# ergodicio/tsadar

Hardware: AMD Instinct MI355X
Metric: spectra/sec (fwd+grad), 1024-lambda EPW+IAW form factor, batch 4096 (higher is better)
Workload: dtype f64

## Files before the change

tsadar_amd/csrc/k_spectrum_fused.inc:

```

template <int NI, int GM, bool ZH, bool FAR = false>
__device__ __forceinline__ double point_fused(const Base& b, const Base& bn, bool has_next, const LineS<NI>& L, const Tables& T,
                                              double PQ, double cw, BaseAdj& ba, double& xen, double& Fn, LineS<NI>& J) {
  PointF<NI> pf;
  point_core<NI, ZH, FAR>(b, bn, has_next, L, T, pf);
  const double ik2 = pf.ik2, ike2 = pf.ike2, vph = pf.vph, gsum = pf.gsum, Wl = pf.Wl, dW = pf.dW, idx = pf.idx, D = pf.D;
  const double cer = pf.cer, cei = pf.cei, opc = pf.opc, cim = pf.cim, er = pf.er, ei = pf.ei, ieps2 = pf.ieps2, ce2 = pf.ce2, ci2 = pf.ci2;
  const double N = pf.N, t1 = pf.t1, S = pf.S, dop = pf.dop;
  const double* xi = pf.xi; const double* zr = pf.zr; const double* zi = pf.zi; const double* dzr = pf.dzr; const double* dzi = pf.dzi;
  const double* hk = pf.hk; const double* gs = pf.gs;
  const double Sb = PQ * dop;
  const double PSQ = PQ * S;
  const double fwd = S * dop;
  J.wL = __builtin_fma(PSQ * b.wd, cw, J.wL);
  const double Nb = Sb * t1;
  const double ikb0 = Sb * N * ieps2;
  const double e2 = -2.0 * (ikb0 * t1);
  const double NbI = Nb * L.ivTe;
  const double ci2b2 = 2.0 * (NbI * b.F);
  ba.F = NbI * ci2;
  J.ivTe += (Nb * ci2) * b.F;
  const double erb = e2 * er, eib = e2 * ei;
  double cerb = erb, ceib = eib, cimb = eib;
  if (!FAR) {
    const double ce2b2 = 2.0 * (Nb * gsum);
    cerb = erb + ce2b2 * cer; ceib = eib + ce2b2 * cei;
    cimb = eib + ci2b2 * cim;
  }
  const double creb = erb + ci2b2 * opc;
  const double cp = ceib * kPi;
  const double ike2b = cp * D - cerb * Wl;
  const double Wlb = -cerb * ike2;
  ba.xe = Wlb * dW;
  if (GM == 1) {
    double Wml, dWm;
    w_lookup(T.Wm, b.xe, Wml, dWm);
    J.m += Wlb * Wml;
  }
  Fn = (cp * ike2) * idx;
  ba.F -= Fn;
  xen = -Fn * D;
  ba.xe -= xen;
  double k2acc = 0.0, vphb = 0.0;
  const double u = FAR ? 0.0 : Nb * ce2;
#pragma unroll
  for (int s = 0; s < NI; ++s) {
    double w, xib;
    if (FAR) {
      w = creb * zr[s];
      xib = hk[s] * (creb * dzr[s]);
    } else {
      const double v = u * gs[s];
      J.cs[s] += v;
      w = creb * zr[s] + cimb * zi[s];
      xib = -2.0 * (v * xi[s] * L.cs[s]) + hk[s] * (creb * dzr[s] + cimb * dzi[s]);
    }
    const double wk = w * ik2;
    J.a_i[s] += wk;
    k2acc += wk * hk[s];
    vphb += xib * L.ixi[s];
    J.ixi[s] += xib * vph;
  }
  const double we = ike2b * ik2;
  J.a_e += we;
  ba.k2 = -k2acc - we * ike2;
  ba.wd = PSQ * L.i2wL + vphb * b.ik;
  ba.ik = ikb0 + vphb * b.wd;
  return fwd;
}

struct KsAcc { double p1a, p2a, p1b, p2b; };

template <int NI, int GM>
__device__ __forceinline__ double base_reverse_fused(const Base& b, const LineS<NI>& L, const Tables& T, const BaseAdj& ba,
                                                     LineS<NI>& LB) {
  const double Hb = ba.F * b.F;
  if (GM == 1) {
    Tables Tm = T;
    Tm.hc = T.hcm;
    double Hm, dHm;
    hermite_lookup_c(Tm, b.xe, Hm, dHm);
    LB.m += (b.xe < T.vx0 || b.xe > T.vxlast) ? 0.0 : Hb * Hm;
  }
  const double xeb = ba.xe + Hb * b.dH;
  const double vph = b.wd * b.ik, k = b.k2 * b.ik;
  const double vphb = xeb * L.ivTe;
  LB.Ud -= vphb;
  LB.ivTe += xeb * (vph - L.Ud);
  const double wdb = ba.wd + vphb * b.ik;
  const double ikb = ba.ik + vphb * b.wd;
  LB.wL -= wdb;
  LB.Vd -= wdb * k;
  const double kb = wdb * L.Vd + ikb * (b.ik * b.ik);
  return 2.0 * ba.k2 - kb * b.ik;
}

template <int NI, int GM>
__device__ __forceinline__ double base_reverse_xf(const Base& b, const LineS<NI>& L, const Tables& T, double xeb_in, double Fb,
                                                  LineS<NI>& LB) {
  const double Hb = Fb * b.F;
  if (GM == 1) {
    Tables Tm = T;
    Tm.hc = T.hcm;
    double Hm, dHm;
    hermite_lookup_c(Tm, b.xe, Hm, dHm);
    LB.m += (b.xe < T.vx0 || b.xe > T.vxlast) ? 0.0 : Hb * Hm;
  }
  const double xeb = xeb_in + Hb * b.dH;
  const double vph = b.wd * b.ik, k = b.k2 * b.ik;
  const double vphb = xeb * L.ivTe;
  LB.Ud -= vphb;
  LB.ivTe += xeb * (vph - L.Ud);
  const double wdb = vphb * b.ik;
  const double ikb = vphb * b.wd;
  LB.wL -= wdb;
  LB.Vd -= wdb * k;
  const double kb = wdb * L.Vd + ikb * (b.ik * b.ik);
  return -kb * b.ik;
}

#ifdef TSFF_TRACE
__device__ unsigned long long* g_trace_buf = nullptr;
#define TSFF_STAMP(k) do { if (tid == 0 && g_trace_buf) g_trace_buf[(size_t)item * 16 + (k)] = wall_clock64(); } while (0)
#define TSFF_STAMP_WAVE(k) do { if (lane == 0 && g_trace_buf) g_trace_buf[(size_t)item * 16 + (k) + hw] = wall_clock64(); } while (0)
#define TSFF_STAMP_HW() do { if (tid == 0 && g_trace_buf) g_trace_buf[(size_t)item * 16] = ((unsigned long long)__builtin_amdgcn_s_getreg(20 | (31 << 11)) << 32) | (unsigned)__builtin_amdgcn_s_getreg(4 | (31 << 11)); } while (0)
#else
#define TSFF_STAMP(k) do {} while (0)
#define TSFF_STAMP_WAVE(k) do {} while (0)
#define TSFF_STAMP_HW() do {} while (0)
#endif
typedef const double __attribute__((address_space(4))) cdouble_t;
template <int DIR>
__device__ __forceinline__ void conv4_phase(const double* __restrict__ xs, int Ls, int sl, cdouble_t* pt, int na, double (&acc)[4]) {
  const double* __restrict__ X0 = xs + sl, * __restrict__ X1 = X0 + Ls, * __restrict__ X2 = X1 + Ls, * __restrict__ X3 = X2 + Ls;
  double V0 = X0[0], V1 = X1[0], V2 = X2[0];
#pragma unroll 2
  for (int a = 0; a < na; ++a) {
    const double V3 = X3[a], V4 = X0[a + 1], V5 = X1[a + 1], V6 = X2[a + 1];
    const double g0 = pt[4 * DIR * a], g1 = pt[4 * DIR * a + DIR], g2 = pt[4 * DIR * a + 2 * DIR], g3 = pt[4 * DIR * a + 3 * DIR];
    acc[0] = __builtin_fma(g3, V3, __builtin_fma(g2, V2, __builtin_fma(g1, V1, __builtin_fma(g0, V0, acc[0]))));
    acc[1] = __builtin_fma(g3, V4, __builtin_fma(g2, V3, __builtin_fma(g1, V2, __builtin_fma(g0, V1, acc[1]))));
    acc[2] = __builtin_fma(g3, V5, __builtin_fma(g2, V4, __builtin_fma(g1, V3, __builtin_fma(g0, V2, acc[2]))));
    acc[3] = __builtin_fma(g3, V6, __builtin_fma(g2, V5, __builtin_fma(g1, V4, __builtin_fma(g0, V3, acc[3]))));
    V0 = V4; V1 = V5; V2 = V6;
  }
}

constexpr int kRedSums = 32;
#ifndef TSFF_FUSED_FAR
#define TSFF_FUSED_FAR 1
#endif
template <int NI, int GM, bool ZH, bool EX = false>
__global__ __launch_bounds__(kHalf, 2) void k_spectrum_fused(KStatic S, KCall K, int f0, int flags,
                                                             const double* __restrict__ lrec) {
  const bool use_ks = flags & 2, interleaved = flags & 4;
  const int item = blockIdx.x;
  const int f_il = interleaved ? (int)(item >= K.B) : 0;
  const int b = K.b0 + item - f_il * K.B, tid = threadIdx.x;
  const size_t gitem = (size_t)f_il * K.Btot + b;
  constexpr int TPF = kHalf, NW = TPF / 64;
  const int ht = tid, lane = tid & 63, hw = tid >> 6;
  const int f = __builtin_amdgcn_readfirstlane(interleaved ? f_il : f0);
  extern __shared__ __align__(16) unsigned char smem[];
  TSFF_STAMP_HW();
  TSFF_STAMP(1);
  const Smem m = carve(smem, S, 1, GM, use_ks, true, ZH, EX);
  constexpr int NPk = TSFF_NP(NI);
  const double* __restrict__ xpar = K.params + (size_t)b * S.NP;
  const int npts = S.npts, NA = S.n_angles;
  const int hs = S.hs, Ls = npts / 4 + 2 * hs;
  double* xs = m.x;
  auto XA = [&](int j) { return (j & 3) * Ls + (j >> 2) + hs; };
  Tables T;
  const double lam_shift = S.lam_shift[f];
  const double* __restrict__ omgs = S.omgs[f];
  constexpr int kPair = 2;
  const int jp[2] = {kPair * ht, npts / 2 + kPair * ht};
  double ws[2][kPair + 1];
  LineS<NI> L;
  double* __restrict__ ksc = use_ks ? m.ksc : nullptr;
  {
    TSFF_STAGE_LOCALS;
    stage_issue(TSFF_STAGE_ARGS, m, S, K, S.shared_fe ? 0 : b, ZH, f);
    stage_commit(TSFF_STAGE_ARGS, m, S, K, S.shared_fe ? 0 : b, T, ZH, f);
#pragma unroll
    for (int p = 0; p < 2; ++p)
#pragma unroll
      for (int q = 0; q <= kPair; ++q) ws[p][q] = omgs[min(jp[p] + q, npts - 1)];
    {
      lines_load<NI>(lrec + gitem * kLineRec, 1, [](double v) { return uni(v); }, L);
    }
    if (use_ks) {
#pragma unroll
      for (int p = 0; p < 2; ++p)
#pragma unroll
        for (int q = 0; q <= kPair; ++q) ksc[min(jp[p] + q, npts - 1)] = ks_eval(ws[p][q], L.wpe2);
    }
    for (int i = ht; i < 8 * hs; i += TPF) { const int ph_ = i / (2 * hs), o = i - ph_ * 2 * hs; xs[ph_ * Ls + (o < hs ? o : Ls - 2 * hs + o)] = 0.0; }
    if (ht < 2) xs[4 * Ls + ht] = 0.0;
  }
  double w_lo[2], w_hi[2];
#pragma unroll
  for (int p = 0; p < 2; ++p) {
    w_lo[p] = __hiloint2double(__builtin_amdgcn_readlane(__double2hiint(ws[p][0]), 0), __builtin_amdgcn_readlane(__double2loint(ws[p][0]), 0));
    w_hi[p] = __hiloint2double(__builtin_amdgcn_readlane(__double2hiint(ws[p][kPair]), 63), __builtin_amdgcn_readlane(__double2loint(ws[p][kPair]), 63));
  }
  const bool far0 = TSFF_FUSED_FAR && far_range_w<NI>(w_lo[0], w_hi[0], L), far1 = TSFF_FUSED_FAR && far_range_w<NI>(w_lo[1], w_hi[1], L);
  const double ex_wse = ((lane >> 4) & 1) ? w_hi[1] : w_hi[0];
  __syncthreads();
  TSFF_STAMP(2);
  auto JQ = [&](int q) { return jp[q >> 1] + (q & 1); };
  LineS<NI> J[kStrip];
  KsAcc KA[kStrip];
  double xa[kStrip];
#pragma unroll
  for (int q = 0; q < kStrip; ++q) { zero_lines<NI>(J[q]); xa[q] = 0.0; KA[q].p1a = KA[q].p2a = KA[q].p1b = KA[q].p2b = 0.0; }
  const double cw = -0.5 * L.i2wL * L.i2wL;
  double* exl = m.ex;
  double* exb = EX ? m.ex + kExComp * kHalf : nullptr;
  if (EX) {
    const int Pb = (lane >> 4) & 1, ab = lane & 15;
    if (lane < 32 && ab < NA) {
      const double wse = ex_wse;
      Base be;
      base_eval<NI>(wse, ks_eval(wse, L.wpe2), m.cosa[ab], L, T, be);
      double* o = exb + 16 * (2 * hw + Pb) + ab;
      o[0] = be.wd; o[kExBound] = be.ik; o[2 * kExBound] = be.xe; o[3 * kExBound] = be.F; o[4 * kExBound] = be.dH;
    }
    __builtin_amdgcn_fence(__ATOMIC_RELEASE, "wavefront");
    __builtin_amdgcn_wave_barrier();
  }
  auto sweep = [&](auto pair_tag, auto far_tag) {
    constexpr int P = decltype(pair_tag)::value;
    constexpr bool FAR = decltype(far_tag)::value;
    const int jb = jp[P];
    const int j2 = min(jb + kPair, npts - 1);
    const double ks2 = EX ? (use_ks ? ksc[j2] : ks_eval(ws[P][kPair], L.wpe2)) : 0.0;
    double ct_n = m.cosa[0], wa_n = m.wsa[0];
    for (int a = 0; a < NA; ++a) {
      const double ct = uni(ct_n), wa = uni(wa_n * L.pref);
      { const int an = min(a + 1, NA - 1); ct_n = m.cosa[an]; wa_n = m.wsa[an]; }
      Base b0;
      base_eval<NI>(ws[P][0], use_ks ? ksc[jb] : ks_eval(ws[P][0], L.wpe2), ct, L, T, b0);
      if (EX) {
        exl[ht] = b0.wd; exl[kHalf + ht] = b0.ik; exl[2 * kHalf + ht] = b0.xe; exl[3 * kHalf + ht] = b0.F; exl[4 * kHalf + ht] = b0.dH;
        __builtin_amdgcn_fence(__ATOMIC_RELEASE, "wavefront");
        __builtin_amdgcn_wave_barrier();
      }
#pragma unroll
      for (int i = 0; i < kPair; ++i) {
        constexpr int q0 = kPair * P;
        const int q = q0 + i, j = jb + i;
        const bool has_next = (j + 1) < npts;
        Base b1;
        if (EX && i == kPair - 1) {
          __builtin_amdgcn_wave_barrier();
          __builtin_amdgcn_fence(__ATOMIC_ACQUIRE, "wavefront");
          const double* src = lane == 63 ? exb + 16 * (2 * hw + P) + a : exl + ht + 1;
          const int cs = lane == 63 ? kExBound : kHalf;
          b1.wd = src[0]; b1.ik = src[cs]; b1.xe = src[2 * cs]; b1.F = src[3 * cs]; b1.dH = src[4 * cs];
          b1.ks = ks2;
          b1.k2 = base_k2<NI>(ks2, ct, L);
          __builtin_amdgcn_wave_barrier();
        } else {
          base_eval<NI>(ws[P][i + 1], use_ks ? ksc[min(j + 1, npts - 1)] : ks_eval(ws[P][i + 1], L.wpe2), ct, L, T, b1);
        }
        BaseAdj ba;
        double xen, Fn;
        xa[q] = __builtin_fma(wa, point_fused<NI, GM, ZH, FAR>(b0, b1, has_next, L, T, wa, cw, ba, xen, Fn, J[q]), xa[q]);
        const double k22a = base_reverse_fused<NI, GM>(b0, L, T, ba, J[q]);
        const double k22b = base_reverse_xf<NI, GM>(b1, L, T, xen, Fn, J[q]);
        KA[q].p1a += k22a; KA[q].p2a = __builtin_fma(k22a, ct, KA[q].p2a);
        KA[q].p1b += k22b; KA[q].p2b = __builtin_fma(k22b, ct, KA[q].p2b);
        b0 = b1;
      }
    }
  };
  if (far0) sweep(std::integral_constant<int, 0>{}, std::true_type{}); else sweep(std::integral_constant<int, 0>{}, std::false_type{});
  if (far1) sweep(std::integral_constant<int, 1>{}, std::true_type{}); else sweep(std::integral_constant<int, 1>{}, std::false_type{});
  TSFF_STAMP_WAVE(9);
#ifdef TSFF_SWEEP_ONLY
  {
    double acc = 0.0;
#pragma unroll
    for (int q = 0; q < kStrip; ++q) acc += xa[q] + J[q].wL + J[q].ivTe + J[q].a_e + J[q].Ud + J[q].Vd + J[q].ixi[0] + J[q].a_i[0] + J[q].cs[0] + KA[q].p1a + KA[q].p2a + KA[q].p1b + KA[q].p2b;
    __syncthreads();
    TSFF_STAMP(3);
    if (acc == 1.2345e300) K.gpart[0] = acc;
    TSFF_STAMP(8);
    return;
  }
#endif
#pragma unroll
  for (int q = 0; q < kStrip; ++q) {
    const int j = JQ(q);
    const double ksa = use_ks ? ksc[j] : ks_eval(ws[q >> 1][q & 1], L.wpe2);
    const double ksb = use_ks ? ksc[min(j + 1, npts - 1)] : ks_eval(ws[q >> 1][(q & 1) + 1], L.wpe2);
    const double p1 = KA[q].p1a + KA[q].p1b;
    J[q].kL = L.kL * p1 - (ksa * KA[q].p2a + ksb * KA[q].p2b);
    J[q].wpe2 = -(0.5 / (kC * kC)) * (p1 - L.kL * (KA[q].p2a / ksa + KA[q].p2b / ksb));
  }
  {
    const bool filt = f == TSFF_FEATURE_ELE && S.filt;
#pragma unroll
    for (int q = 0; q < kStrip; ++q) {
      const double w = ws[q >> 1][q & 1];
      xs[XA(JQ(q))] = xa[q] * (filt ? w * w * S.filt[JQ(q)] : w * w);
    }
  }
  __syncthreads();
  TSFF_STAMP(3);

  constexpr int BPT = 4;
  typedef const double __attribute__((address_space(4))) cdouble;
  const bool raw = S.raw[f];
  const size_t row4 = (size_t)b * TSFF_NBINS + 4 * ht;
  double dpre[BPT], npre[BPT], lpre[BPT];
  uint8_t mpre[BPT];
#pragma unroll
  for (int r = 0; r < BPT; ++r) {
    dpre[r] = K.data[f][row4 + r];
    npre[r] = K.noise[f] ? K.noise[f][row4 + r] : 0.0;
    lpre[r] = f == TSFF_FEATURE_ELE ? S.lam_bin[f][4 * ht + r] : 0.0;
    mpre[r] = S.mask[f][4 * ht + r];
  }
  const double amps = raw ? 1.0 : K.amps[f][b];
  const double* __restrict__ lrp = lrec + gitem * kLineRec + 9 + 4 * NI;
  const double p_lam_v = lrp[0], p_amp1_v = lrp[1], p_amp2_v = lrp[2], p_amp3_v = lrp[3];
  double wpre[BPT];
  {
    const bool filt = f == TSFF_FEATURE_ELE && S.filt;
#pragma unroll
    for (int r = 0; r < BPT; ++r) {
      const double w = omgs[4 * ht + r];
      wpre[r] = filt ? w * w * S.filt[4 * ht + r] : w * w;
    }
  }
  double ybin[BPT] = {0.0, 0.0, 0.0, 0.0};
  conv4_phase<1>(xs, Ls, ht + S.cf_a0[f] + hs, (cdouble_t*)(S.ptaps[f] + S.cf_i0[f]), S.cf_na[f], ybin);
  double M = ybin[0];
  int pstar = 4 * ht;
#pragma unroll
  for (int r = 1; r < BPT; ++r)
    if (ybin[r] > M) { M = ybin[r]; pstar = 4 * ht + r; }
  half_argmax<NW>(M, pstar, m.red, 0, hw, lane);
  TSFF_STAMP(4);
  const double invM = raw ? 1.0 : 1.0 / M;
  const double p_lam = uni(p_lam_v), p_amp1 = uni(p_amp1_v), p_amp2 = uni(p_amp2_v), p_amp3 = uni(p_amp3_v);
  double Tb[BPT], Ap[BPT];
  double s0 = 0.0, s1 = 0.0;
#pragma unroll
  for (int r = 0; r < BPT; ++r) {
    const int pb = 4 * ht + r;
    const double A = bin_amplitude(f, raw, amps, lpre[r], p_lam, p_amp1, p_amp2, p_amp3);
    Ap[r] = A;
    const double t = thry_value(A, ybin[r], invM, K.noise[f] != nullptr, npre[r]);
    if (K.thry[f]) K.thry[f][(size_t)b * TSFF_NBINS + pb] = t;
    Tb[r] = bin_loss(S, K, f, dpre[r], t, mpre[r], s0, s1);
  }

  double sn = 0.0, a1b = 0.0, a2b = 0.0;
#pragma unroll
  for (int r = 0; r < BPT; ++r) norm_adjoint_bin(f, Tb[r], ybin[r], invM, Ap[r], amps, lpre[r], p_lam, sn, a1b, a2b);
  {
    double v5[5] = {s0, s1, sn, a1b, a2b};
#pragma unroll
    for (int k = 0; k < 5; ++k) v5[k] = wave_sum(v5[k]);
    if (lane == 0) {
#pragma unroll
      for (int k = 0; k < 5; ++k) m.red[kRedSums + k * NW + hw] = v5[k];
    }
  }
#pragma unroll
  for (int r = 0; r < BPT; ++r) xs[XA(4 * ht + r)] = Tb[r] * Ap[r] * invM;
  __syncthreads();
  TSFF_STAMP(5);
  double sx[4] = {0.0, 0.0, 0.0, 0.0};
  conv4_phase<-1>(xs, Ls, ht + S.ca_a0[f] + hs, (cdouble_t*)(S.ptaps[f] + S.ca_i0[f]), S.ca_na[f], sx);

  __syncthreads();
  TSFF_STAMP(6);
  {
    const double* r = m.red + kRedSums;
    s0 = (r[0] + r[1]) + (r[2] + r[3]);
    s1 = (r[NW] + r[NW + 1]) + (r[NW + 2] + r[NW + 3]);
    sn = (r[2 * NW] + r[2 * NW + 1]) + (r[2 * NW + 2] + r[2 * NW + 3]);
    a1b = (r[3 * NW] + r[3 * NW + 1]) + (r[3 * NW + 2] + r[3 * NW + 3]);
    a2b = (r[4 * NW] + r[4 * NW + 1]) + (r[4 * NW + 2] + r[4 * NW + 3]);
  }
  if (ht == 0) {
    if (f == TSFF_FEATURE_ELE) { K.lpart[(size_t)b * 3 + 1] = s0; K.lpart[(size_t)b * 3 + 2] = s1; }
    else K.lpart[(size_t)b * 3 + 0] = s0;
  }
  if (raw) sn = a1b = a2b = 0.0;
  {
    const bool filt = f == TSFF_FEATURE_ELE && S.filt;
    const double cn = sn * invM;
    const int s_first = 4 * ht - pstar - S.toff[f], nt = S.ntaps[f];
#pragma unroll
    for (int r = 0; r < 4; ++r) {
      const int i = 4 * ht + r, st = s_first + r;
      const double xb = (st >= 0 && st < nt) ? __builtin_fma(-cn, m.taps[3 + st], sx[r]) : sx[r];
      xs[XA(i)] = xb * wpre[r];
    }
  }
  __syncthreads();
  constexpr int NLB = 9 + 3 * NI;
  LineS<NI> LB;
  zero_lines<NI>(LB);
#pragma unroll
  for (int q = 0; q < kStrip; ++q) {
    const double xb = xs[XA(JQ(q))];
    LB.wpe2 += xb * J[q].wpe2; LB.wL += xb * J[q].wL; LB.kL += xb * J[q].kL; LB.ivTe += xb * J[q].ivTe;
    LB.a_e += xb * J[q].a_e; LB.Ud += xb * J[q].Ud; LB.Vd += xb * J[q].Vd; LB.m += xb * J[q].m;
    LB.pref += xb * xa[q];
#pragma unroll
    for (int s = 0; s < NI; ++s) { LB.ixi[s] += xb * J[q].ixi[s]; LB.a_i[s] += xb * J[q].a_i[s]; LB.cs[s] += xb * J[q].cs[s]; }
  }
  LB.pref *= 1.0 / L.pref;
#pragma unroll
  for (int s = 0; s < NI; ++s) LB.a_i[s] *= -0.5;
  {
    double lb[kLBRec];
    lines_adj_store<NI>(LB, lb);
#pragma unroll
    for (int k = 0; k < NLB; ++k) lb[k] = wave_sum(lb[k]);
    lb[NLB] = a1b; lb[NLB + 1] = a2b;
    const size_t nitems = (size_t)K.Btot * (interleaved ? 2 : 1);
    double mine = 0.0;
#pragma unroll
    for (int k = 0; k < NLB + 2; ++k) mine = lane == k ? lb[k] : mine;
    if (lane < NLB + 2) K.lbrec[((size_t)lane * NW + hw) * nitems + gitem] = mine;
  }
  TSFF_STAMP(8);
}

template <int NI>
__global__ __launch_bounds__(64) void k_fused_prep(KStatic S, const double* __restrict__ params, int B, int f0, int nload,
                                                   double* __restrict__ lrec, double* __restrict__ finrec) {
  constexpr int NPk = TSFF_NP(NI);
  const int item = blockIdx.x * 64 + threadIdx.x;
  if (item >= B * nload) return;
  const size_t nitems = (size_t)B * nload;
  const int l = item / B, b = item - l * B, f = nload == 2 ? l : f0;
  const double* __restrict__ x = params + (size_t)b * S.NP;
  double sgv[NPk];
#pragma unroll
  for (int s = 0; s < NPk; ++s) sgv[s] = S.p_sig[s] ? sigmoid(x[s]) : 0.0;
  Phys<NI> p;
  load_phys<NI>(x, S.p_scale, S.p_shift, S.p_sig, S.ti_same, true, p, sgv);
  LineS<NI> L;
  make_lines<NI>(p, S.lam_shift[f], 0, 1, L);
  {
    double ph[NPk + 1];
    phys_to_array<NI>(p, ph);
    double* __restrict__ q = finrec + item;
#pragma unroll
    for (int k = 0; k <= NPk; ++k) q[(size_t)k * nitems] = ph[k];
#pragma unroll
    for (int k = 0; k < NPk; ++k) q[(size_t)(NPk + 1 + k) * nitems] = sgv[k];
    lines_store<NI>(L, q + (size_t)(2 * NPk + 1) * nitems, nitems);
  }
  double* __restrict__ r = lrec + (size_t)item * kLineRec;
  lines_store<NI>(L, r, 1);
  r[9 + 4 * NI] = p.lam; r[10 + 4 * NI] = p.amp1; r[11 + 4 * NI] = p.amp2; r[12 + 4 * NI] = p.amp3;
}

template <int NI>
__global__ __launch_bounds__(kThreads) void k_fused_finish(KStatic S, const double* __restrict__ finrec, const double* __restrict__ lbrec,
                                                     const double* __restrict__ lpart, int B, int f0, int nload, int gm,
                                                     const uint8_t* __restrict__ gmask, double* __restrict__ grad,
                                                     double* __restrict__ loss_out, const int* __restrict__ act, int n_act,
                                                     long B_global, long b_off, double* __restrict__ packed) {
  constexpr int NPk = TSFF_NP(NI), NLB = 9 + 3 * NI, NW = kHalf / 64;
  __shared__ double red[8];
  const int lane = threadIdx.x;
  const int per_wg = kThreads / nload;
  if (blockIdx.x == gridDim.x - 1) {
    double a[3] = {0.0, 0.0, 0.0};
    constexpr int U = 8;
    for (int b0 = threadIdx.x; b0 < B; b0 += U * kThreads) {
      double v[U][3];
#pragma unroll
      for (int u = 0; u < U; ++u) {
        const int bb = b0 + u * kThreads;
#pragma unroll
        for (int k = 0; k < 3; ++k) v[u][k] = bb < B ? lpart[(size_t)bb * 3 + k] : 0.0;
      }
#pragma unroll
      for (int u = 0; u < U; ++u)
        if (b0 + u * kThreads < B) { a[0] += v[u][0]; a[1] += v[u][1]; a[2] += v[u][2]; }
    }
    double* out = packed ? packed : loss_out;
    for (int k = 0; k < 3; ++k) {
      const double v = block_sum(a[k], red);
      if (threadIdx.x == 0) out[k] = v;
    }
    return;
  }
  const int b = blockIdx.x * per_wg + lane / nload, l = nload == 2 ? (lane & 1) : 0;
  int actv[NPk];
#pragma unroll
  for (int k = 0; k < NPk; ++k) actv[k] = (packed && k < n_act) ? act[k] : -1;
  const size_t nitems = (size_t)B * nload;
  double gv[NPk];
#pragma unroll
  for (int s = 0; s < NPk; ++s) gv[s] = 0.0;
  if (b < B) {
    const int f = nload == 2 ? l : f0;
    const size_t item = (size_t)l * B + b;
    const double* __restrict__ q = finrec + item;
    double ph[NPk + 1], sgv[NPk];
#pragma unroll
    for (int k = 0; k <= NPk; ++k) ph[k] = q[(size_t)k * nitems];
#pragma unroll
    for (int k = 0; k < NPk; ++k) sgv[k] = q[(size_t)(NPk + 1 + k) * nitems];
    Phys<NI> p;
    phys_from_lds<NI>(ph, p);
    q += (size_t)(2 * NPk + 1) * nitems;
    LineS<NI> L;
    lines_load<NI>(q, nitems, [](double v) { return v; }, L);
    double lb[NLB];
#pragma unroll
    for (int k = 0; k < NLB; ++k) {
      const double* __restrict__ r = lbrec + (size_t)k * NW * nitems + item;
      lb[k] = (r[0] + r[nitems]) + (r[2 * nitems] + r[3 * nitems]);
    }
    const double a1b = lbrec[(size_t)NLB * NW * nitems + item], a2b = lbrec[(size_t)(NLB + 1) * NW * nitems + item];
    LineS<NI> LB;
    zero_lines<NI>(LB);
    lines_adj_load<NI>(lb, true, LB);
    double g[NPk];
#pragma unroll
    for (int s = 0; s < NPk; ++s) g[s] = 0.0;
    make_lines_adjoint<NI>(p, S.lam_shift[f], 0, 1, L, LB, g);
    amp_adjoint(f, a1b, a2b, g);
    tie_renorm_adjoint<NI>(S, p, gm == 1, g);
#pragma unroll
    for (int s = 0; s < NPk; ++s) gv[s] = activation_adjoint(g[s], S.p_scale[s], S.p_sig[s], [&] { return sgv[s]; }, gmask[s]);
  }
  if (nload == 2) {
#pragma unroll
    for (int s = 0; s < NPk; ++s) {
      const double o = __shfl_xor(gv[s], 1, 64);
      gv[s] = (lane & 1) ? 0.0 : gv[s] + o;
    }
  }
  if (b < B && l == 0) {
    if (packed) {
#pragma unroll
      for (int k = 0; k < NPk; ++k) {
        double v = 0.0;
#pragma unroll
        for (int s = 0; s < NPk; ++s) v = actv[k] == s ? gv[s] : v;
        if (actv[k] >= 0) packed[3 + (size_t)k * B_global + b_off + b] = v;
      }
    } else {
#pragma unroll
      for (int s = 0; s < NPk; ++s) grad[(size_t)b * NPk + s] = gv[s];
    }
  }
  if (packed) {
    const long n = (long)n_act * B_global;
    if ((long)B < B_global)
      for (long i = (long)blockIdx.x * kThreads + lane; i < n; i += (long)(gridDim.x - 1) * kThreads) {
        const long k = i / B_global, bl = i - k * B_global - b_off;
        if (bl < 0 || bl >= B) packed[3 + i] = 0.0;
      }
  }
}
```

tsadar_amd/csrc/tsff_device.h:

```cpp
#pragma once
#include <hip/hip_runtime.h>
#include <stdint.h>
#include <type_traits>

#include "../../include/tsff.h"

#ifndef TSFF_BRANCHFREE
#define TSFF_BRANCHFREE 1
#endif

namespace tsff {

constexpr int kThreads = 256;
constexpr int kStrip = 4;
constexpr int kNP_MAX = TSFF_NP(TSFF_MAX_ION);

constexpr double kC = 2.99792458e10;
constexpr double kMe = 510.9896 / (kC * kC);
constexpr double kMp = kMe * 1836.1;
constexpr double kRe = 2.8179e-13;
constexpr double kPi = 3.14159265358979323846;
constexpr double kEsq = kMe * kC * kC * kRe;
constexpr double kC0sq = 4.0 * kPi * kEsq / kMe;
constexpr double kOmgLnum = 2.0 * kPi * 1e7 * kC;
constexpr double kInvSqrt2Pi = 0.39894228040143267794;
constexpr double kSqrt2 = 1.41421356237309504880;

constexpr double kXi2_0 = -8.2;
constexpr double kXi2_h = 0.01;
constexpr double kXi2_ih = 100.0;
constexpr int kNXi2 = TSFF_NXI2;
constexpr int kNXi1 = TSFF_NXI1;

#ifndef TSFF_NEWTON
#define TSFF_NEWTON 1
#endif
__device__ __forceinline__ double frcp(double x) {
  double y = __builtin_amdgcn_rcp(x);
  double e = __builtin_fma(-x, y, 1.0);
  y = __builtin_fma(y, e, y);
#if TSFF_NEWTON > 1
  e = __builtin_fma(-x, y, 1.0);
  y = __builtin_fma(y, e, y);
#endif
  return y;
}

__device__ __forceinline__ void fsqrt2(double x, double& s, double& is) {
  const double y = __builtin_amdgcn_rsq(x);
  double g = x * y, h = 0.5 * y;
  double r = __builtin_fma(-h, g, 0.5);
  g = __builtin_fma(g, r, g);
  h = __builtin_fma(h, r, h);
#if TSFF_NEWTON > 1
  r = __builtin_fma(-h, g, 0.5);
  g = __builtin_fma(g, r, g);
  h = __builtin_fma(h, r, h);
#endif
  const double d = __builtin_fma(-g, g, x);
  s = __builtin_fma(d, h, g);
  is = h + h;
}

__device__ __forceinline__ double uni(double x) {
  const int lo = __builtin_amdgcn_readfirstlane(__double2loint(x));
  const int hi = __builtin_amdgcn_readfirstlane(__double2hiint(x));
  return __hiloint2double(hi, lo);
}

__device__ __forceinline__ double wave_sum(double v) {
#pragma unroll
  for (int o = 32; o > 0; o >>= 1) v += __shfl_xor(v, o, 64);
  return v;
}

__device__ __forceinline__ double block_sum(double v, double* scratch) {
  v = wave_sum(v);
  const int lane = threadIdx.x & 63, w = threadIdx.x >> 6;
  __syncthreads();
  if (lane == 0) scratch[w] = v;
  __syncthreads();
  return (scratch[0] + scratch[1]) + (scratch[2] + scratch[3]);
}

__device__ __forceinline__ void block_argmax(double& v, int& idx, double* scratch) {
#pragma unroll
  for (int o = 32; o > 0; o >>= 1) {
    double ov = __shfl_xor(v, o, 64);
    int oi = __shfl_xor(idx, o, 64);
    if (ov > v || (ov == v && oi < idx)) { v = ov; idx = oi; }
  }
  const int lane = threadIdx.x & 63, w = threadIdx.x >> 6;
  __syncthreads();
  if (lane == 0) { scratch[w] = v; scratch[4 + w] = (double)idx; }
  __syncthreads();
  v = scratch[0]; idx = (int)scratch[4];
#pragma unroll
  for (int k = 1; k < 4; ++k) {
    double ov = scratch[k]; int oi = (int)scratch[4 + k];
    if (ov > v || (ov == v && oi < idx)) { v = ov; idx = oi; }
  }
}

struct Tables {
  const double2* zp;
  const double* W;
  const double2* ht;
  const double2* hc;
  const double2* hcm;
  const double* Wm;
  double* Wb;
  double* Hy;
  double* Hs;
  double vx0, dv, idv, vxlast;
  double u0, utop;
  const double* etab;
  int nvx;
};
__device__ __forceinline__ void tables_set_grid(Tables& T, double vx0, double dv, int nvx) {
  T.vx0 = vx0; T.dv = dv; T.idv = 1.0 / dv; T.vxlast = vx0 + (nvx - 1) * dv; T.nvx = nvx;
  T.u0 = -vx0 * T.idv; T.utop = (double)(nvx - 1) * (1.0 - 1.1102230246251565e-16);
}

struct FeAcc {
  int iw, ih;
  double w0, w1, y0, y1, s0, s1;
};
__device__ __forceinline__ void fe_acc_init(FeAcc& a) { a.iw = a.ih = -1; a.w0 = a.w1 = a.y0 = a.y1 = a.s0 = a.s1 = 0.0; }
__device__ __forceinline__ void fe_flush_w(FeAcc& a, double* Wb) {
  if (a.iw >= 0) { atomicAdd(&Wb[a.iw], a.w0); atomicAdd(&Wb[a.iw + 1], a.w1); }
  a.w0 = a.w1 = 0.0;
}
__device__ __forceinline__ void fe_flush_h(FeAcc& a, double* Hy, double* Hs) {
  if (a.ih >= 0) {
    atomicAdd(&Hy[a.ih], a.y0); atomicAdd(&Hy[a.ih + 1], a.y1);
    atomicAdd(&Hs[a.ih], a.s0); atomicAdd(&Hs[a.ih + 1], a.s1);
  }
  a.y0 = a.y1 = a.s0 = a.s1 = 0.0;
}
__device__ __forceinline__ void fe_add_w(FeAcc& a, double* Wb, double xe, double wb) {
  const double xlast = kXi2_0 + (kNXi2 - 1) * kXi2_h;
  const double u = (xe - kXi2_0) * kXi2_ih;
  int i = (int)u;
  i = i < 0 ? 0 : (i > kNXi2 - 2 ? kNXi2 - 2 : i);
  double t = (xe - (kXi2_0 + i * kXi2_h)) * kXi2_ih;
  t = xe < kXi2_0 ? 0.0 : (xe > xlast ? 1.0 : t);
  if (i != a.iw) { fe_flush_w(a, Wb); a.iw = i; }
  a.w0 += wb * (1.0 - t);
  a.w1 += wb * t;
}
__device__ __forceinline__ void fe_add_h(FeAcc& a, const Tables& T, double x, double hb) {
  if (x < T.vx0 || x > T.vxlast) return;
  const double u = (x - T.vx0) * T.idv;
  int i = (int)u;
  i = i < 0 ? 0 : (i > T.nvx - 2 ? T.nvx - 2 : i);
  const double t = (x - (T.vx0 + i * T.dv)) * T.idv;
  if (i != a.ih) { fe_flush_h(a, T.Hy, T.Hs); a.ih = i; }
  const double t2 = t * t, t3 = t2 * t;
  a.y0 += hb * (2.0 * t3 - 3.0 * t2 + 1.0);
  a.y1 += hb * (3.0 * t2 - 2.0 * t3);
  a.s0 += hb * (t3 - 2.0 * t2 + t) * T.dv;
  a.s1 += hb * (t3 - t2) * T.dv;
}

__device__ __forceinline__ void w_lookup(const double* W, double xe, double& w, double& dw) {
#pragma clang fp contract(off)
  constexpr double kTop = (double)(kNXi2 - 1) * (1.0 - 1.1102230246251565e-16);
  const double u = __builtin_fma(xe, kXi2_ih, -kXi2_0 * kXi2_ih);
  const double uc = fmin(fmax(u, 0.0), kTop);
  const double fl = __builtin_floor(uc);
  const double t = uc - fl;
  const int i = (int)fl;
  const double a = W[i], b = W[i + 1];
  const double d = b - a;
  w = __builtin_fma(t, d, a);
  dw = (u == uc) ? d * kXi2_ih : 0.0;
}

__device__ __forceinline__ void hermite_coeffs(double2 a, double2 b, double dv, double2& c01, double2& c23) {
  const double f0 = a.x, f1 = b.x, m0 = a.y * dv, m1 = b.y * dv;
  c01 = make_double2(f0, m0);
  c23 = make_double2(-3.0 * f0 + 3.0 * f1 - 2.0 * m0 - m1, 2.0 * f0 - 2.0 * f1 + m0 + m1);
}

__device__ __forceinline__ void hermite_lookup_c(const Tables& T, double x, double& H, double& dH) {
#pragma clang fp contract(off)
  const double u = __builtin_fma(x, T.idv, T.u0);
  const double uc = fmin(fmax(u, 0.0), T.utop);
  const double fl = __builtin_floor(uc);
  const double t = uc - fl;
  const int i = (int)fl;
  const double2 c01 = T.hc[2 * i], c23 = T.hc[2 * i + 1];
  const bool out = u != uc;
  const double Hi = __builtin_fma(t, __builtin_fma(t, __builtin_fma(t, c23.y, c23.x), c01.y), c01.x);
  const double dHi = __builtin_fma(t, __builtin_fma(3.0 * t, c23.y, 2.0 * c23.x), c01.y) * T.idv;
  H = out ? -50.0 : Hi;
  dH = out ? 0.0 : dHi;
}

__device__ __forceinline__ void hermite_lookup(const Tables& T, double x, double& H, double& dH) {
  double u = (x - T.vx0) * T.idv;
  int i = (int)u;
  i = i < 0 ? 0 : (i > T.nvx - 2 ? T.nvx - 2 : i);
  const double t = (x - (T.vx0 + i * T.dv)) * T.idv;
  const double2 a = T.ht[i], b = T.ht[i + 1];
  const double f0 = a.x, f1 = b.x, m0 = a.y * T.dv, m1 = b.y * T.dv;
  const double c2 = -3.0 * f0 + 3.0 * f1 - 2.0 * m0 - m1;
  const double c3 = 2.0 * f0 - 2.0 * f1 + m0 + m1;
  if (x < T.vx0 || x > T.vxlast) { H = -50.0; dH = 0.0; }
  else {
    H = f0 + t * (m0 + t * (c2 + t * c3));
    dH = (m0 + t * (2.0 * c2 + 3.0 * t * c3)) * T.idv;
  }
}

template <int NI>
struct Phys {
  double Te, ne, m, lam, amp1, amp2, amp3, neg, teg, ud, Va;
  double Ti[NI], Z[NI], A[NI], fr[NI];
  double fsum;
};

template <int NI>
struct LineS {
  double wpe2, wL, kL, ivTe, a_e, pref, Ud, Vd;
  double i2wL;
  double m;
  double ixi[NI], a_i[NI], cs[NI];
  double hai[NI];
};

__device__ __forceinline__ double grad_coef(int g, int G) {
  return G == 1 ? -1.0 / 200.0 : -1.0 / 200.0 + (double)g / (100.0 * (double)(G - 1));
}

template <int NI>
__device__ __forceinline__ void make_lines(const Phys<NI>& p, double lam_shift, int g, int G, LineS<NI>& L) {
  const double cg = grad_coef(g, G);
  const double ne_g = 1.0e20 * p.ne * (1.0 + p.neg * cg);
  const double Te_g = p.Te * (1.0 + p.teg * cg);
  L.wL = kOmgLnum / (p.lam + lam_shift);
  L.i2wL = 2.0 / L.wL;
  L.m = 0.0;
  L.wpe2 = kC0sq * ne_g;
  L.kL = sqrt(L.wL * L.wL - L.wpe2) / kC;
  L.ivTe = 1.0 / sqrt(Te_g / kMe);
  L.a_e = L.wpe2 * L.ivTe * L.ivTe;
  L.pref = kRe * kRe * ne_g / (2.0 * kPi * kC);
  L.Ud = p.ud * 1e6;
  L.Vd = p.Va * 1e6;
  double Zbar = 0.0;
#pragma unroll
  for (int s = 0; s < NI; ++s) Zbar += p.Z[s] * p.fr[s];
#pragma unroll
  for (int s = 0; s < NI; ++s) {
    const double Ms = p.A[s] * kMp;
    const double vTi = sqrt(p.Ti[s] / Ms);
    L.ixi[s] = 1.0 / (kSqrt2 * vTi);
    L.a_i[s] = kC0sq * kMe * p.Z[s] * p.Z[s] * p.fr[s] * ne_g / (Zbar * p.Ti[s]);
    L.cs[s] = p.fr[s] * p.Z[s] * p.Z[s] / (Zbar * vTi);
    L.hai[s] = -0.5 * L.a_i[s];
  }
}

template <int NI>
__device__ __forceinline__ void make_lines_uniform(const Phys<NI>& p, double lam_shift, int g, int G, LineS<NI>& L) {
  make_lines<NI>(p, lam_shift, g, G, L);
  L.wpe2 = uni(L.wpe2); L.wL = uni(L.wL); L.i2wL = uni(L.i2wL); L.kL = uni(L.kL); L.ivTe = uni(L.ivTe);
  L.a_e = uni(L.a_e); L.pref = uni(L.pref); L.Ud = uni(L.Ud); L.Vd = uni(L.Vd);
#pragma unroll
  for (int s = 0; s < NI; ++s) { L.ixi[s] = uni(L.ixi[s]); L.a_i[s] = uni(L.a_i[s]); L.cs[s] = uni(L.cs[s]); L.hai[s] = uni(L.hai[s]); }
}

template <int NI>
__device__ __forceinline__ void make_lines_adjoint(const Phys<NI>& p, double lam_shift, int g, int G,
                                                   const LineS<NI>& L, const LineS<NI>& LB, double* pb) {
  const double cg = grad_coef(g, G);
  const double gfn = 1.0 + p.neg * cg, gft = 1.0 + p.teg * cg;
  const double ne_g = 1.0e20 * p.ne * gfn;
  const double Te_g = p.Te * gft;
  double wpe2b = LB.wpe2, wLb = LB.wL, ivTeb = LB.ivTe;
  double ne_gb = LB.pref * (kRe * kRe / (2.0 * kPi * kC));
  wpe2b += LB.a_e * L.ivTe * L.ivTe;
  ivTeb += LB.a_e * 2.0 * L.wpe2 * L.ivTe;
  wLb += LB.kL * L.wL / (kC * kC * L.kL);
  wpe2b += LB.kL * (-0.5 / (kC * kC * L.kL));
  double Zbar = 0.0;
#pragma unroll
  for (int s = 0; s < NI; ++s) Zbar += p.Z[s] * p.fr[s];
  double Zbarb = 0.0;
#pragma unroll
  for (int s = 0; s < NI; ++s) {
    const double Ms = p.A[s] * kMp;
    const double vTi = sqrt(p.Ti[s] / Ms);
    const double Z2 = p.Z[s] * p.Z[s];
    double Tib = 0.0, Zb = 0.0, frb = 0.0;
    const double ai_over_fr = kC0sq * kMe * Z2 * ne_g / (Zbar * p.Ti[s]);
    Zb += LB.a_i[s] * 2.0 * L.a_i[s] / p.Z[s];
    frb += LB.a_i[s] * ai_over_fr;
    ne_gb += LB.a_i[s] * L.a_i[s] / ne_g;
    Zbarb -= LB.a_i[s] * L.a_i[s] / Zbar;
    Tib -= LB.a_i[s] * L.a_i[s] / p.Ti[s];
    Tib += LB.ixi[s] * (-0.5 * L.ixi[s] / p.Ti[s]);
    Tib += LB.cs[s] * (-0.5 * L.cs[s] / p.Ti[s]);
    Zb += LB.cs[s] * 2.0 * L.cs[s] / p.Z[s];
    frb += LB.cs[s] * Z2 / (Zbar * vTi);
    Zbarb -= LB.cs[s] * L.cs[s] / Zbar;
    pb[TSFF_P_ION0 + 4 * s + TSFF_ION_TI] += Tib;
    pb[TSFF_P_ION0 + 4 * s + TSFF_ION_Z] += Zb;
    pb[TSFF_P_ION0 + 4 * s + TSFF_ION_FRACT] += frb;
  }
#pragma unroll
  for (int s = 0; s < NI; ++s) {
    pb[TSFF_P_ION0 + 4 * s + TSFF_ION_Z] += Zbarb * p.fr[s];
    pb[TSFF_P_ION0 + 4 * s + TSFF_ION_FRACT] += Zbarb * p.Z[s];
  }
  const double Te_gb = ivTeb * (-0.5 * L.ivTe / Te_g);
  ne_gb += wpe2b * kC0sq;
  const double lam0 = p.lam + lam_shift;
  pb[TSFF_P_LAM] += wLb * (-L.wL / lam0);
  pb[TSFF_P_NE] += ne_gb * 1.0e20 * gfn;
  pb[TSFF_P_NE_GRADIENT] += ne_gb * 1.0e20 * p.ne * cg;
  pb[TSFF_P_TE] += Te_gb * gft;
  pb[TSFF_P_TE_GRADIENT] += Te_gb * p.Te * cg;
  pb[TSFF_P_UD] += LB.Ud * 1e6;
  pb[TSFF_P_VA] += LB.Vd * 1e6;
  pb[TSFF_P_M] += LB.m;
}


#ifndef TSFF_FEXP
#define TSFF_FEXP 1
#endif
template <bool CLAMP = true>
__device__ __forceinline__ double fexp(double x) {
#if !TSFF_FEXP
  return exp(x);
#endif
  if (CLAMP) x = fmax(x, -800.0);
  const double n = __builtin_rint(x * 1.4426950408889634074);
  double r = __builtin_fma(n, -6.93147180369123816490e-01, x);
  r = __builtin_fma(n, -1.90821492927058770002e-10, r);
#if TSFF_FEXP == 1
  double p = 1.6059043836821613e-10;
  p = __builtin_fma(p, r, 2.08767569878681e-09);
  p = __builtin_fma(p, r, 2.505210838544172e-08);
  p = __builtin_fma(p, r, 2.755731922398589e-07);
  p = __builtin_fma(p, r, 2.7557319223985893e-06);
  p = __builtin_fma(p, r, 2.48015873015873e-05);
  p = __builtin_fma(p, r, 1.984126984126984e-04);
  p = __builtin_fma(p, r, 1.388888888888889e-03);
  p = __builtin_fma(p, r, 8.333333333333333e-03);
  p = __builtin_fma(p, r, 4.1666666666666664e-02);
  p = __builtin_fma(p, r, 1.6666666666666666e-01);
  p = __builtin_fma(p, r, 0.5);
  p = __builtin_fma(p, r, 1.0);
  p = __builtin_fma(p, r, 1.0);
#elif TSFF_FEXP == 2
  double p = 2.505210838544172e-08;
  p = __builtin_fma(p, r, 2.755731922398589e-07);
  p = __builtin_fma(p, r, 2.7557319223985893e-06);
  p = __builtin_fma(p, r, 2.48015873015873e-05);
  p = __builtin_fma(p, r, 1.984126984126984e-04);
  p = __builtin_fma(p, r, 1.388888888888889e-03);
  p = __builtin_fma(p, r, 8.333333333333333e-03);
  p = __builtin_fma(p, r, 4.1666666666666664e-02);
  p = __builtin_fma(p, r, 1.6666666666666666e-01);
  p = __builtin_fma(p, r, 0.5);
  p = __builtin_fma(p, r, 1.0);
  p = __builtin_fma(p, r, 1.0);
// ... 409 lines not shown
```

Baseline: 4.725 million.

## Software-pipeline conv4 tap and LDS loads with double-buffered registers

Rewrites the 4-wide convolution loop so the next pair of iterations' scalar tap loads and LDS window loads are issued before computing the current pair. Explicit lgkmcnt waits and sched barriers enforce the ordering, with two register buffers alternating. Also hoists the filter, noise and lambda pointer selection so the per-bin loads become unconditional, and adds a trace stamp. This raises register pressure at 2 blocks per SM launch bounds and fixes the schedule by hand instead of leaving it to the compiler.

```diff
diff --git a/tsadar_amd/csrc/k_spectrum_fused.inc b/tsadar_amd/csrc/k_spectrum_fused.inc
--- a/tsadar_amd/csrc/k_spectrum_fused.inc
+++ b/tsadar_amd/csrc/k_spectrum_fused.inc
@@ -129,23 +129,6 @@
 #define TSFF_STAMP_WAVE(k) do {} while (0)
 #define TSFF_STAMP_HW() do {} while (0)
 #endif
-typedef const double __attribute__((address_space(4))) cdouble_t;
-template <int DIR>
-__device__ __forceinline__ void conv4_phase(const double* __restrict__ xs, int Ls, int sl, cdouble_t* pt, int na, double (&acc)[4]) {
-  const double* __restrict__ X0 = xs + sl, * __restrict__ X1 = X0 + Ls, * __restrict__ X2 = X1 + Ls, * __restrict__ X3 = X2 + Ls;
-  double V0 = X0[0], V1 = X1[0], V2 = X2[0];
-#pragma unroll 2
-  for (int a = 0; a < na; ++a) {
-    const double V3 = X3[a], V4 = X0[a + 1], V5 = X1[a + 1], V6 = X2[a + 1];
-    const double g0 = pt[4 * DIR * a], g1 = pt[4 * DIR * a + DIR], g2 = pt[4 * DIR * a + 2 * DIR], g3 = pt[4 * DIR * a + 3 * DIR];
-    acc[0] = __builtin_fma(g3, V3, __builtin_fma(g2, V2, __builtin_fma(g1, V1, __builtin_fma(g0, V0, acc[0]))));
-    acc[1] = __builtin_fma(g3, V4, __builtin_fma(g2, V3, __builtin_fma(g1, V2, __builtin_fma(g0, V1, acc[1]))));
-    acc[2] = __builtin_fma(g3, V5, __builtin_fma(g2, V4, __builtin_fma(g1, V3, __builtin_fma(g0, V2, acc[2]))));
-    acc[3] = __builtin_fma(g3, V6, __builtin_fma(g2, V5, __builtin_fma(g1, V4, __builtin_fma(g0, V3, acc[3]))));
-    V0 = V4; V1 = V5; V2 = V6;
-  }
-}
-
 constexpr int kRedSums = 32;
 #ifndef TSFF_FUSED_FAR
 #define TSFF_FUSED_FAR 1
@@ -291,6 +274,11 @@
     return;
   }
 #endif
+  const bool filt = f == TSFF_FEATURE_ELE && S.filt;
+  const double* __restrict__ fsrc = filt ? S.filt : omgs;
+  double fq[kStrip];
+#pragma unroll
+  for (int q = 0; q < kStrip; ++q) fq[q] = fsrc[JQ(q)];
 #pragma unroll
   for (int q = 0; q < kStrip; ++q) {
     const int j = JQ(q);
@@ -301,11 +289,10 @@
     J[q].wpe2 = -(0.5 / (kC * kC)) * (p1 - L.kL * (KA[q].p2a / ksa + KA[q].p2b / ksb));
   }
   {
-    const bool filt = f == TSFF_FEATURE_ELE && S.filt;
 #pragma unroll
     for (int q = 0; q < kStrip; ++q) {
       const double w = ws[q >> 1][q & 1];
-      xs[XA(JQ(q))] = xa[q] * (filt ? w * w * S.filt[JQ(q)] : w * w);
+      xs[XA(JQ(q))] = xa[q] * (filt ? w * w * fq[q] : w * w);
     }
   }
   __syncthreads();
@@ -315,27 +302,25 @@
   typedef const double __attribute__((address_space(4))) cdouble;
   const bool raw = S.raw[f];
   const size_t row4 = (size_t)b * TSFF_NBINS + 4 * ht;
+  const double* __restrict__ dsrc = K.data[f];
+  const double* __restrict__ noise = K.noise[f];
+  const double* __restrict__ nsrc = noise ? noise : dsrc;
+  const double* __restrict__ lsrc = f == TSFF_FEATURE_ELE ? S.lam_bin[f] : omgs;
   double dpre[BPT], npre[BPT], lpre[BPT];
   uint8_t mpre[BPT];
 #pragma unroll
   for (int r = 0; r < BPT; ++r) {
-    dpre[r] = K.data[f][row4 + r];
-    npre[r] = K.noise[f] ? K.noise[f][row4 + r] : 0.0;
-    lpre[r] = f == TSFF_FEATURE_ELE ? S.lam_bin[f][4 * ht + r] : 0.0;
+    dpre[r] = dsrc[row4 + r];
+    npre[r] = nsrc[row4 + r];
+    lpre[r] = lsrc[4 * ht + r];
     mpre[r] = S.mask[f][4 * ht + r];
   }
   const double amps = raw ? 1.0 : K.amps[f][b];
   const double* __restrict__ lrp = lrec + gitem * kLineRec + 9 + 4 * NI;
   const double p_lam_v = lrp[0], p_amp1_v = lrp[1], p_amp2_v = lrp[2], p_amp3_v = lrp[3];
-  double wpre[BPT];
-  {
-    const bool filt = f == TSFF_FEATURE_ELE && S.filt;
-#pragma unroll
-    for (int r = 0; r < BPT; ++r) {
-      const double w = omgs[4 * ht + r];
-      wpre[r] = filt ? w * w * S.filt[4 * ht + r] : w * w;
-    }
-  }
+  double wpw[BPT], wpf[BPT];
+#pragma unroll
+  for (int r = 0; r < BPT; ++r) { wpw[r] = omgs[4 * ht + r]; wpf[r] = fsrc[4 * ht + r]; }
   double ybin[BPT] = {0.0, 0.0, 0.0, 0.0};
   conv4_phase<1>(xs, Ls, ht + S.cf_a0[f] + hs, (cdouble_t*)(S.ptaps[f] + S.cf_i0[f]), S.cf_na[f], ybin);
   double M = ybin[0];
@@ -354,7 +339,7 @@
     const int pb = 4 * ht + r;
     const double A = bin_amplitude(f, raw, amps, lpre[r], p_lam, p_amp1, p_amp2, p_amp3);
     Ap[r] = A;
-    const double t = thry_value(A, ybin[r], invM, K.noise[f] != nullptr, npre[r]);
+    const double t = thry_value(A, ybin[r], invM, noise != nullptr, npre[r]);
     if (K.thry[f]) K.thry[f][(size_t)b * TSFF_NBINS + pb] = t;
     Tb[r] = bin_loss(S, K, f, dpre[r], t, mpre[r], s0, s1);
   }
@@ -394,14 +379,14 @@
   }
   if (raw) sn = a1b = a2b = 0.0;
   {
-    const bool filt = f == TSFF_FEATURE_ELE && S.filt;
     const double cn = sn * invM;
     const int s_first = 4 * ht - pstar - S.toff[f], nt = S.ntaps[f];
 #pragma unroll
     for (int r = 0; r < 4; ++r) {
       const int i = 4 * ht + r, st = s_first + r;
       const double xb = (st >= 0 && st < nt) ? __builtin_fma(-cn, m.taps[3 + st], sx[r]) : sx[r];
-      xs[XA(i)] = xb * wpre[r];
+      const double w = wpw[r];
+      xs[XA(i)] = xb * (filt ? w * w * wpf[r] : w * w);
     }
   }
   __syncthreads();
@@ -420,6 +405,7 @@
   LB.pref *= 1.0 / L.pref;
 #pragma unroll
   for (int s = 0; s < NI; ++s) LB.a_i[s] *= -0.5;
+  TSFF_STAMP(7);
   {
     double lb[kLBRec];
     lines_adj_store<NI>(LB, lb);
diff --git a/tsadar_amd/csrc/tsff_device.h b/tsadar_amd/csrc/tsff_device.h
--- a/tsadar_amd/csrc/tsff_device.h
+++ b/tsadar_amd/csrc/tsff_device.h
@@ -66,6 +66,52 @@
   const int lo = __builtin_amdgcn_readfirstlane(__double2loint(x));
   const int hi = __builtin_amdgcn_readfirstlane(__double2hiint(x));
   return __hiloint2double(hi, lo);
+}
+
+typedef const double __attribute__((address_space(4))) cdouble_t;
+__device__ __forceinline__ void conv4_group(double g0, double g1, double g2, double g3, double& V0, double& V1, double& V2, double V3,
+                                            double V4, double V5, double V6, double (&acc)[4]) {
+  acc[0] = __builtin_fma(g3, V3, __builtin_fma(g2, V2, __builtin_fma(g1, V1, __builtin_fma(g0, V0, acc[0]))));
+  acc[1] = __builtin_fma(g3, V4, __builtin_fma(g2, V3, __builtin_fma(g1, V2, __builtin_fma(g0, V1, acc[1]))));
+  acc[2] = __builtin_fma(g3, V5, __builtin_fma(g2, V4, __builtin_fma(g1, V3, __builtin_fma(g0, V2, acc[2]))));
+  acc[3] = __builtin_fma(g3, V6, __builtin_fma(g2, V5, __builtin_fma(g1, V4, __builtin_fma(g0, V3, acc[3]))));
+  V0 = V4; V1 = V5; V2 = V6;
+}
+constexpr unsigned kWaitLgkm0 = 0xC07F;
+template <int DIR>
+__device__ __forceinline__ void conv4_phase(const double* __restrict__ xs, int Ls, int sl, cdouble_t* pt, int na, double (&acc)[4]) {
+  const double* __restrict__ X0 = xs + sl, * __restrict__ X1 = X0 + Ls, * __restrict__ X2 = X1 + Ls, * __restrict__ X3 = X2 + Ls;
+  double V0 = X0[0], V1 = X1[0], V2 = X2[0];
+  int a = 0;
+  if (na & 1) {
+    conv4_group(pt[0], pt[DIR], pt[2 * DIR], pt[3 * DIR], V0, V1, V2, X3[0], X0[1], X1[1], X2[1], acc);
+    a = 1;
+  }
+  if (a >= na) return;
+  auto request = [&](int a_, double (&g)[8], double (&w)[8]) {
+#pragma unroll
+    for (int k = 0; k < 8; ++k) g[k] = pt[DIR * (4 * a_ + k)];
+    w[0] = X3[a_]; w[1] = X0[a_ + 1]; w[2] = X1[a_ + 1]; w[3] = X2[a_ + 1];
+    w[4] = X3[a_ + 1]; w[5] = X0[a_ + 2]; w[6] = X1[a_ + 2]; w[7] = X2[a_ + 2];
+  };
+  double gA[8], wA[8], gB[8], wB[8];
+  request(a, gA, wA);
+  for (;;) {
+    __builtin_amdgcn_s_waitcnt(kWaitLgkm0);
+    __builtin_amdgcn_sched_barrier(0);
+    request(min(a + 2, na - 2), gB, wB);
+    conv4_group(gA[0], gA[1], gA[2], gA[3], V0, V1, V2, wA[0], wA[1], wA[2], wA[3], acc);
+    conv4_group(gA[4], gA[5], gA[6], gA[7], V0, V1, V2, wA[4], wA[5], wA[6], wA[7], acc);
+    a += 2;
+    if (a >= na) break;
+    __builtin_amdgcn_s_waitcnt(kWaitLgkm0);
+    __builtin_amdgcn_sched_barrier(0);
+    request(min(a + 2, na - 2), gA, wA);
+    conv4_group(gB[0], gB[1], gB[2], gB[3], V0, V1, V2, wB[0], wB[1], wB[2], wB[3], acc);
+    conv4_group(gB[4], gB[5], gB[6], gB[7], V0, V1, V2, wB[4], wB[5], wB[6], wB[7], acc);
+    a += 2;
+    if (a >= na) break;
+  }
 }
 
 __device__ __forceinline__ double wave_sum(double v) {
```

Result: faster. 4.779 million, median of 6 (+1.1%).
